# phuang1024/Starst3r

Hardware: AMD Instinct MI355X
Metric: 3DGS train iters/sec @ 1M Gaussians, 8x1080p views (higher is better)
Workload: dtype f32

## Files before the change

### starst3r_amd/csrc/api.hip

```cpp
#include <stdarg.h>

#include "common.h"

static thread_local char g_err[512] = "";

void st3r_set_error(const char* fmt, ...) {
    va_list ap;
    va_start(ap, fmt);
    vsnprintf(g_err, sizeof(g_err), fmt, ap);
    va_end(ap);
}

ST3R_EXPORT int st3r_version(void) { return ST3R_VERSION; }
ST3R_EXPORT const char* st3r_last_error(void) { return g_err; }

ST3R_EXPORT int st3r_ctx_create(int device, st3r_ctx** out) {
    ARG_CHECK(out);
    int ndev = 0;
    HIP_TRY(hipGetDeviceCount(&ndev));
    ARG_CHECK(device >= 0 && device < ndev);
    HIP_TRY(hipSetDevice(device));
    st3r_ctx* c = new (std::nothrow) st3r_ctx();
    if (!c) { st3r_set_error("out of host memory"); return ST3R_ERR_NOMEM; }
    memset(c, 0, sizeof(*c));
// ... 43 lines not shown
    *grown = 0;
    if (bytes == 0) bytes = 16;
    if (ctx->slot_bytes[slot] < bytes) {
        size_t want = bytes + bytes / 4;
        want = (want + 255) & ~(size_t)255;
        if (ctx->slot_ptr[slot]) {
            HIP_TRY(hipDeviceSynchronize());
            HIP_TRY(hipFree(ctx->slot_ptr[slot]));
            ctx->slot_ptr[slot] = nullptr; ctx->slot_bytes[slot] = 0;
        }
        hipError_t e = hipMalloc(&ctx->slot_ptr[slot], want);
        if (e != hipSuccess) {
            st3r_set_error("arena slot %d: hipMalloc(%zu) failed: %s", slot, want, hipGetErrorString(e));
            return ST3R_ERR_NOMEM;
        }
        ctx->slot_bytes[slot] = want;
        *grown = 1;
    }
    *out = ctx->slot_ptr[slot];
    return ST3R_OK;
}

ST3R_EXPORT int st3r_ctx_peek(st3r_ctx* ctx, void* stream, int which, void* dst, int64_t bytes) {
    ARG_CHECK(ctx && dst && bytes >= 0 && which >= 0 && which <= 10);
    static const int slots[11] = {SLOT_VALS_B, SLOT_OFFSETS, SLOT_SPLATS, SLOT_CUM,
                                  SLOT_MCMC_CUM, SLOT_MCMC_DEAD, SLOT_MCMC_SAMPLED, SLOT_MCMC_COUNT,
                                  SLOT_RGB, SLOT_ALPHA, SLOT_COUNTS};
    ARG_CHECK((size_t)bytes <= ctx->slot_bytes[slots[which]]);
    HIP_TRY(hipMemcpyAsync(dst, ctx->slot_ptr[slots[which]], (size_t)bytes, hipMemcpyDeviceToDevice,
                           (hipStream_t)stream));
    return ST3R_OK;
}

static const char* k_stage_names[STG_COUNT] = {"project", "scan", "emit", "sort", "offsets", "blend_fwd", "loss",
                                               "blend_bwd", "project_bwd", "adam", "sort_depth"};

ST3R_EXPORT const char* st3r_stage_name(int stage) {
    return (stage >= 0 && stage < STG_COUNT) ? k_stage_names[stage] : "";
}

static void prof_harvest_slot(st3r_ctx* ctx, int slot) {
    for (int st = 0; st < STG_COUNT; ++st) {
        if (!ctx->prof_used[slot][st]) continue;
        float ms = 0.f;
        if (hipEventSynchronize(ctx->prof_ev[slot][st][1]) == hipSuccess &&
            hipEventElapsedTime(&ms, ctx->prof_ev[slot][st][0], ctx->prof_ev[slot][st][1]) == hipSuccess) {
            ctx->prof_ms[st] += ms; ctx->prof_n[st] += 1;
        }
        ctx->prof_used[slot][st] = 0;
    }
// ... 57 lines not shown
int st3r_project_impl(st3r_ctx* ctx, hipStream_t s, int N, int C, const float* means, const float* quats, const float* scales,
                      const float* opacities, const float* sh, int sh_stride, const float* viewmats, const float* Ks,
                      const float* campos, int width, int height, int tile_size, float eps2d, float near_plane,
                      float far_plane, float radius_clip, float* splats, int32_t* tiles_per_gauss, double* reg_sums,
                      uint64_t* depth_keys, int32_t* depth_vals, int tight, uint32_t key_base, void* rects, int rect32,
                      int reg_overwrite, double* zero_ptr, int zero_n, uint32_t* krange);
int st3r_sort_depth_seg_impl(st3r_ctx* ctx, hipStream_t s, int64_t N, int C, uint32_t* keys_in, int32_t* vals_in,
                             uint32_t* keys_out, int32_t* vals_out, const uint32_t* krange);
int st3r_isect_emit_chain_impl(st3r_ctx* ctx, hipStream_t s, int N, int C, const int32_t* perm, const void* rects,
                               int rect32, int tile_w, int tile_h, uint32_t* tile_keys, int32_t* vals, int64_t cap);
int st3r_records_prepare_impl(hipStream_t s, int N, int C, const float* splats, int tile_size, int tile_w, int tile_h,
                              int tight, int32_t* tiles, uint64_t* depth_keys, int32_t* depth_vals, uint32_t key_base,
                              void* rects, int rect32);
int st3r_isect_offsets32_impl(hipStream_t s, int64_t n_isects, const uint32_t* keys, int C, int tile_w, int tile_h,
                              int32_t* offsets, const int32_t* n_dev);
int st3r_sort_depth_impl(st3r_ctx* ctx, hipStream_t s, int64_t n, int end_bit, uint64_t* keys_in, int32_t* vals_in,
                         uint64_t* keys_out, int32_t* vals_out);
int st3r_sort_depth32_impl(st3r_ctx* ctx, hipStream_t s, int64_t n, int end_bit, uint32_t* keys_in, int32_t* vals_in,
                           uint32_t* keys_out, int32_t* vals_out);
int st3r_sort_tile_impl(st3r_ctx* ctx, hipStream_t s, int64_t n, int end_bit, uint32_t* keys_in, int32_t* vals_in,
                        uint32_t* keys_out, int32_t* vals_out, const int32_t* n_dev);
int st3r_blend_fwd_impl(st3r_ctx* ctx, hipStream_t s, int C, int W, int H, int tile_w, int tile_h,
                        const float* splats, const int32_t* offsets, const int32_t* flat, int64_t n_isects,
                        float* rgb, float* alpha, int32_t* last_ids, bool for_backward, bool end_in_offsets);
int st3r_blend_bwd_impl(st3r_ctx* ctx, hipStream_t s, int C, int W, int H, int tile_w, int tile_h,
                        const float* splats, const int32_t* offsets, const int32_t* flat, int64_t n_isects,
                        const float* alpha, const int32_t* last_ids, const float* v_rgb, const float* v_alpha,
                        const int32_t* cum, const uint64_t* rects, const uint64_t* rectbase, int tight, int64_t n_pairs,
                        float* v_splats,
                        bool end_in_offsets, st3r_vtile_ref* defer);
int st3r_project_sh_bwd_impl(hipStream_t s, int N, int C, const float* means, const float* quats, const float* scales,
                             const float* opacities, const float* sh, int sh_stride, const float* viewmats,
                             const float* Ks, const float* campos, int width, int height, float eps2d,
                             const float* splats, const float* v_splats, float reg_views, float opac_fac,
                             float scale_fac, float* grads, bool accumulate, int g_begin, int g_end, bool range_major,
                             const st3r_vtile_ref* slots);
int st3r_loss_impl(st3r_ctx* ctx, hipStream_t s, int C, int H, int W, const float* render, const float* gt,
                   float w_l1, float w_ssim, double* sums, float* v_render, bool sums_cleared);

static int bit_length_u32(uint32_t v) { int n = 0; while (v) { ++n; v >>= 1; } return n; }

static int settle_pending_count(st3r_ctx* ctx) {
    if (!ctx->count_pending) return ST3R_OK;
    HIP_TRY(hipEventSynchronize(ctx->count_event));
    ctx->count_pending = 0;
    const int64_t n = (int64_t)((int32_t*)(ctx->pinned + 8))[0];
    if (n < 0) {
        ctx->isect_hint = 0;
        ctx->view_chunks = (ctx->view_chunks > 0 ? ctx->view_chunks : 1) * 2;
        st3r_set_error("the previous step produced more than 2^31 tile intersections: its gradients were incomplete -- "
                       "repeat it (st3r_gs_train_fwd_bwd / st3r_gs_train_step now walk the views in %d chunks)",
                       ctx->view_chunks);
        return ST3R_ERR_CAPACITY;
// ... 173 lines not shown
        for (int c = 0; c < C; ++c) loss += w_l1 * sums[2 * c] * inv_px + w_ssim * (1.0 - sums[2 * c + 1] * inv_cnt);
        loss += reg_views * (opac_k * reg_sums[0] + scale_k * reg_sums[1]);
        loss_out[0] = (float)loss;
    }
}

static int train_views(st3r_ctx* ctx, hipStream_t s, int N, int C, const float* means, const float* quats,
                       const float* scales, const float* opacities, const float* sh, int sh_stride,
                       const float* viewmats, const float* Ks, const float* campos, const float* gt_images, int W, int H,
                       float ssim_fac, float opac_fac, float scale_fac, double* sums, double* reg_sums, bool allow_async,
                       bool accumulate, float* grads, RasterOut* ro_out) {
    const int64_t n_pairs = (int64_t)N * C, n_px = (int64_t)C * H * W;
    RasterOut ro;
    int rc = rasterize_front(ctx, s, N, C, means, quats, scales, opacities, sh, sh_stride, viewmats, Ks, campos, W, H,
                             reg_sums, 1, nullptr, allow_async, &ro, sums);
    if (rc) return rc;
    const bool eio = true;
    GET(SLOT_RGB, float, n_px * 3, rgb);
    GET(SLOT_ALPHA, float, n_px, alpha);
    GET(SLOT_LAST, int32_t, n_px, last);
    GET(SLOT_VRENDER, float, n_px * 3, v_rgb);
    float* const v_splats = nullptr;
    st3r_vtile_ref slots_{}; st3r_vtile_ref* const slots = &slots_;
    st3r_prof_begin(ctx, s, STG_BLEND_FWD);
    rc = st3r_blend_fwd_impl(ctx, s, C, W, H, ro.tile_w, ro.tile_h, ro.splats, ro.offsets, ro.flat, ro.n_isects, rgb,
                             alpha, last, true, eio);
    st3r_prof_end(ctx, s, STG_BLEND_FWD);
    if (rc) return rc;
    st3r_prof_begin(ctx, s, STG_LOSS);
    rc = st3r_loss_impl(ctx, s, C, H, W, rgb, gt_images, 1.0f - ssim_fac, ssim_fac, sums, v_rgb, true);
    st3r_prof_end(ctx, s, STG_LOSS);
    if (rc) return rc;
    st3r_prof_begin(ctx, s, STG_BLEND_BWD);
    rc = st3r_blend_bwd_impl(ctx, s, C, W, H, ro.tile_w, ro.tile_h, ro.splats, ro.offsets, ro.flat, ro.n_isects, alpha,
                             last, v_rgb, nullptr, ro.cum, (ctx->debug_flags & 2) ? nullptr : ro.rects,
                             (ctx->debug_flags & 2) ? nullptr : ro.rectbase, 1, n_pairs, v_splats,
                             eio, slots);
    st3r_prof_end(ctx, s, STG_BLEND_BWD);
    if (rc) return rc;
    st3r_prof_begin(ctx, s, STG_PROJECT_BWD);
    ctx->ranges_recorded = 0;
    if (ctx->n_ranges > 1 && ctx->comm_stream) {
        GET(SLOT_GSTAGE, float, (int64_t)23 * N, gstage);
        const int K = ctx->n_ranges;
        for (int j = 0; j < K && !rc; ++j) {
            const int g0 = (int)((int64_t)N * j / K), g1 = (int)((int64_t)N * (j + 1) / K);
            rc = st3r_project_sh_bwd_impl(s, N, C, means, quats, scales, opacities, sh, sh_stride, viewmats, Ks, campos, W,
                                          H, 0.3f, ro.splats, v_splats, (float)C, opac_fac, scale_fac, gstage, accumulate, g0,
                                          g1, true, slots);
            if (!rc) HIP_TRY(hipEventRecord(ctx->ev_range_bwd[j], s));
        }
        if (!rc) ctx->ranges_recorded = K;
    } else {
        rc = st3r_project_sh_bwd_impl(s, N, C, means, quats, scales, opacities, sh, sh_stride, viewmats, Ks, campos, W, H,
                                      0.3f, ro.splats, v_splats, (float)C, opac_fac, scale_fac, grads, accumulate, 0, -1,
                                      false, slots);
    }
    st3r_prof_end(ctx, s, STG_PROJECT_BWD);
    *ro_out = ro;
    return rc;
// ... 65 lines not shown
    ARG_CHECK(ctx && N > 0 && C > 0 && width > 0 && height > 0 && records && gt_images && v_records && loss_out);
    ARG_CHECK(C <= ST3R_MAX_VIEWS && (int64_t)N * C < 2147483647LL);
    hipStream_t s = (hipStream_t)stream;
    const int W = width, H = height;
    const int64_t n_pairs = (int64_t)N * C, n_px = (int64_t)C * H * W;
    GET(SLOT_SMALL, double, 2 * (size_t)C + 8, small);
    double* sums = small;
    double* reg_sums = small + 2 * C;
    HIP_TRY(hipMemsetAsync(reg_sums, 0, sizeof(double) * 4, s));
    st3r_prof_next_step(ctx);
    RasterOut ro;
    int rc = settle_pending_count(ctx);
    if (rc) return rc;
    rc = rasterize_front(ctx, s, N, C, nullptr, nullptr, nullptr, nullptr, nullptr, 0, nullptr, nullptr, nullptr, W, H,
                         nullptr, 1, records, stats_host == nullptr, &ro);
    if (rc == ST3R_SPLIT_VIEWS) rc = ST3R_ERR_INVALID;
    if (rc) return rc;
    GET(SLOT_RGB, float, n_px * 3, rgb);
    GET(SLOT_ALPHA, float, n_px, alpha);
    GET(SLOT_LAST, int32_t, n_px, last);
    GET(SLOT_VRENDER, float, n_px * 3, v_rgb);
    st3r_prof_begin(ctx, s, STG_BLEND_FWD);
    rc = st3r_blend_fwd_impl(ctx, s, C, W, H, ro.tile_w, ro.tile_h, ro.splats, ro.offsets, ro.flat, ro.n_isects, rgb,
                             alpha, last, true, true);
    st3r_prof_end(ctx, s, STG_BLEND_FWD);
    if (rc) return rc;
    st3r_prof_begin(ctx, s, STG_LOSS);
    rc = st3r_loss_impl(ctx, s, C, H, W, rgb, gt_images, 1.0f - ssim_fac, ssim_fac, sums, v_rgb, false);
    st3r_prof_end(ctx, s, STG_LOSS);
    if (rc) return rc;
    st3r_prof_begin(ctx, s, STG_BLEND_BWD);
    rc = st3r_blend_bwd_impl(ctx, s, C, W, H, ro.tile_w, ro.tile_h, ro.splats, ro.offsets, ro.flat, ro.n_isects, alpha,
                             last, v_rgb, nullptr, ro.cum, ro.rects, ro.rectbase, 1, n_pairs, v_records, true, nullptr);
    st3r_prof_end(ctx, s, STG_BLEND_BWD);
    if (rc) return rc;
    const int Hi = H - 10, Wi = W - 10;
    const double cnt = (Hi > 0 && Wi > 0) ? (double)Hi * Wi * 3 : 0.0;
    hipLaunchKernelGGL(k_finalize_loss, dim3(1), dim3(64), 0, s, C, sums, reg_sums, 1.0 / ((double)H * W * 3),
                       cnt > 0 ? 1.0 / cnt : 0.0, (double)(1.0f - ssim_fac), (double)ssim_fac, 0.0, 0.0, 0.0, loss_out);
    LAUNCH_CHECK();
    if (stats_host) {
        stats_host[0] = -1; stats_host[1] = ro.n_records; stats_host[2] = st3r_ctx_arena_bytes(ctx); stats_host[3] = -1;
    }
    return ST3R_OK;
}

ST3R_EXPORT int st3r_gs_render(st3r_ctx* ctx, void* stream, int N, int C, const float* means, const float* quats,
                               const float* scales, const float* opacities, const float* sh, int sh_stride,
                               const float* viewmats, const float* Ks, const float* campos, int width, int height,
                               float* rgb, float* alpha, int64_t* stats_host) {
    ARG_CHECK(ctx && N > 0 && C > 0 && width > 0 && height > 0 && sh_stride >= 12);
    ARG_CHECK(C <= ST3R_MAX_VIEWS && (int64_t)N * C < 2147483647LL);
    ARG_CHECK(means && quats && scales && opacities && sh && viewmats && Ks && campos && rgb && alpha);
    hipStream_t s = (hipStream_t)stream;
    RasterOut ro;
    int rc = settle_pending_count(ctx);
    if (rc) return rc;
    rc = rasterize_front(ctx, s, N, C, means, quats, scales, opacities, sh, sh_stride, viewmats, Ks, campos, width, height,
                         nullptr, 0, nullptr, false, &ro);
    if (rc == ST3R_SPLIT_VIEWS) rc = ST3R_ERR_INVALID;
    if (rc) return rc;
    GET(SLOT_LAST, int32_t, (int64_t)C * height * width, last);
    rc = st3r_blend_fwd_impl(ctx, s, C, width, height, ro.tile_w, ro.tile_h, ro.splats, ro.offsets, ro.flat,
                             ro.n_isects, rgb, alpha, last, false, true);
    if (rc) return rc;
    if (stats_host) {
        stats_host[0] = -1; stats_host[1] = ro.n_records; stats_host[2] = st3r_ctx_arena_bytes(ctx); stats_host[3] = 0;
    }
    return ST3R_OK;
}
```

### starst3r_amd/csrc/common.h

```cpp
#pragma once
#include <hip/hip_runtime.h>
#include <stdint.h>
#include <stdio.h>
#include <string.h>

#include "../../include/st3r.h"

#define ST3R_EXPORT extern "C" __attribute__((visibility("default")))

void st3r_set_error(const char* fmt, ...);

#define HIP_TRY(expr)                                                                              \
    do {                                                                                           \
        hipError_t _e = (expr);                                                                    \
        if (_e != hipSuccess) {                                                                    \
            st3r_set_error("%s:%d: %s -> %s", __FILE__, __LINE__, #expr, hipGetErrorString(_e));   \
            return ST3R_ERR_HIP;                                                                   \
        }                                                                                          \
    } while (0)

#define ARG_CHECK(cond)                                                                    \
    do {                                                                                   \
        if (!(cond)) {                                                                     \
            st3r_set_error("%s:%d: invalid argument: %s", __FILE__, __LINE__, #cond);      \
// ... 28 lines not shown
    SLOT_DKEYS_B,
    SLOT_DVALS_A,
    SLOT_DVALS_B,
    SLOT_CUM_D,
    SLOT_NN_PART,
    SLOT_MCMC_CUM,
    SLOT_MCMC_DEAD,
    SLOT_MCMC_RANK,
    SLOT_MCMC_COUNT,
    SLOT_MCMC_SAMPLED,
    SLOT_MCMC_BINOMS,
    SLOT_REG_PART,
    SLOT_RECTS,
    SLOT_RECTS_D,
    SLOT_RECTBASE,
    SLOT_COUNTS,
    SLOT_PSTAGE,
    SLOT_GSTAGE,
    SLOT_ALIGN_CTL,
    SLOT_PAIR_TOUCH,
    SLOT_KRANGE_PART,
    SLOT_SCAN_CHAIN,
    SLOT_POSE_PART,
    SLOT_COUNT
};

enum Stage {
    STG_PROJECT = 0,
    STG_SCAN,
    STG_EMIT,
    STG_SORT,
    STG_OFFSETS,
    STG_BLEND_FWD,
    STG_LOSS,
    STG_BLEND_BWD,
    STG_PROJECT_BWD,
    STG_ADAM,
    STG_SORT_DEPTH,
    STG_COUNT
};
#define PROF_RING 64
#define ST3R_MAX_RANGES 8

#define ST3R_SPLIT_VIEWS 1000

struct st3r_vtile_ref { const int32_t* cum; const float* vtile; int stamp; unsigned vt_cap; const uint32_t* touch; };
// ... 44 lines not shown
```

### starst3r_amd/csrc/gs_blend.hip

```cpp
#include <type_traits>

#include "common.h"
#include "tile_rect.h"
#include "blend_common.h"



struct TileGeom {
    int lb, cam, i, j, start, end, tx0, ty0;
    bool inside;
    float px, py;
};

__device__ __forceinline__ TileGeom tile_geom(int C, int W, int H, int tile_w, int tile_h,
                                              const int32_t* __restrict__ offsets, int n_isects) {
    TileGeom g;
    const int n_tiles = tile_w * tile_h, total = C * n_tiles;
        g.lb = xcd_remap(blockIdx.x, total, XCD_GROUP(C, n_tiles, tile_w));
    g.cam = g.lb / n_tiles;
    const int tile = g.lb - g.cam * n_tiles;
    const int ty = tile / tile_w, tx = tile - ty * tile_w;
    g.tx0 = tx * 16; g.ty0 = ty * 16;
    const int w = threadIdx.x >> 6, lane = threadIdx.x & 63;
    g.j = g.tx0 + ((w & 1) << 3) + (lane & 7);
// ... 118 lines not shown
        out_rgb[3 * p] = r; out_rgb[3 * p + 1] = gg; out_rgb[3 * p + 2] = b;
        out_alpha[p] = 1.0f - T;
        last_ids[p] = TRAIN ? (cur == 0x7fffffff ? cur : cur - 1) : cur;
    }
    if (tile_nb && threadIdx.x == 0) tile_nb[g.lb] = nb;
}

static int hand_off_buffers(st3r_ctx* ctx, int C, int tile_w, int tile_h, int64_t n_isects, uint64_t** cmask,
                            int64_t* words, int32_t** tile_nb) {
    const int64_t total = (int64_t)C * tile_w * tile_h;
    *words = (n_isects >> 6) + 4 * total + 8;
    void* p;
    int rc = st3r_arena_get(ctx, SLOT_CMASK, sizeof(uint64_t) * 4 * (size_t)*words, &p);
    if (rc) return rc;
    *cmask = (uint64_t*)p;
    rc = st3r_arena_get(ctx, SLOT_TILE_NB, sizeof(int32_t) * (size_t)total, &p);
    if (rc) return rc;
    *tile_nb = (int32_t*)p;
    return ST3R_OK;
}

int st3r_blend_fwd_cells_impl(st3r_ctx* ctx, hipStream_t s, int C, int W, int H, int tile_w, int tile_h,
                              const float* splats, const int32_t* offsets, const int32_t* flat, float* rgb, float* alpha,
                              int32_t* last_ids, uint64_t* cmask, int64_t cmask_words, int32_t* tile_nb);

int st3r_blend_fwd_impl(st3r_ctx* ctx, hipStream_t s, int C, int W, int H, int tile_w, int tile_h,
                        const float* splats, const int32_t* offsets, const int32_t* flat, int64_t n_isects,
                        float* rgb, float* alpha, int32_t* last_ids, bool for_backward, bool end_in_offsets) {
    const int total = C * tile_w * tile_h;
    uint64_t* cmask = nullptr; int64_t words = 0; int32_t* tile_nb = nullptr;
    if (for_backward) {
        int rc = hand_off_buffers(ctx, C, tile_w, tile_h, n_isects, &cmask, &words, &tile_nb);
        if (rc) return rc;
    }
    if ((for_backward && end_in_offsets && !(ctx->debug_flags & 128)) || (end_in_offsets && (ctx->debug_flags & 512)))
        return st3r_blend_fwd_cells_impl(ctx, s, C, W, H, tile_w, tile_h, splats, offsets, flat, rgb, alpha, last_ids, cmask,
                                         words, tile_nb);
    if (for_backward && end_in_offsets)
        hipLaunchKernelGGL(k_blend_fwd<true>, dim3(total), dim3(BLK), 0, s, C, W, H, tile_w, tile_h, (const float4*)splats,
                           offsets, flat, -1, rgb, alpha, last_ids, cmask, words, tile_nb, ctx->debug_flags & 1);
    else
        hipLaunchKernelGGL(k_blend_fwd<false>, dim3(total), dim3(BLK), 0, s, C, W, H, tile_w, tile_h, (const float4*)splats,
                           offsets, flat, end_in_offsets ? -1 : (int)n_isects, rgb, alpha, last_ids, cmask, words, tile_nb,
                           ctx->debug_flags & 1);
    LAUNCH_CHECK();
    return ST3R_OK;
}

ST3R_EXPORT int st3r_gs_blend_fwd(st3r_ctx* ctx, void* stream, int C, int width, int height, int tile_size,
                                  int tile_w, int tile_h, const float* splats, const int32_t* offsets,
                                  const int32_t* flatten_ids, int64_t n_isects, float* rgb, float* alpha,
                                  int32_t* last_ids) {
    ARG_CHECK(ctx && C > 0 && width > 0 && height > 0 && tile_size == 16);
    ARG_CHECK(tile_w == (width + 15) / 16 && tile_h == (height + 15) / 16);
    ARG_CHECK(splats && offsets && rgb && alpha && last_ids && n_isects >= 0 && n_isects < 2147483647LL);
    ARG_CHECK(n_isects == 0 || flatten_ids);
    return st3r_blend_fwd_impl(ctx, (hipStream_t)stream, C, width, height, tile_w, tile_h, splats, offsets,
                               flatten_ids, n_isects, rgb, alpha, last_ids, true, false);
}

__device__ __forceinline__ void bwd_phase2(const float2* __restrict__ pr, unsigned tpack, int cnt, int lane, const float4* sA, float* accw, float qxf_lane, float qyf_lane,
                                           const float (&pvr)[CHUNK], const float (&pvg)[CHUNK],
                                           const float (&pvb)[CHUNK]) {
    static_assert(CHUNK == 4, "one DPP row per record of the chunk");
    const int r = lane >> 4, part = lane & 15;
    wave_lds_sync();
    const int t = (tpack >> (8 * r)) & 0xFF;
    const float2 mean = *reinterpret_cast<const float2*>(&sA[t]);
    const float dy = mean.y - qyf_lane;
    const float2* src = pr + r * PAIR_STRIDE + PAIR_AT(part * CHUNK);
    float W0 = 0.f, W1 = 0.f, W2 = 0.f, Sr = 0.f, Sg = 0.f, Sb = 0.f;
#pragma unroll
    for (int i = 0; i < CHUNK; ++i) {
        const float2 v = src[i];
        W0 += v.x;
        if (i == 1) { W1 = v.x; W2 = v.x; }
        if (i > 1) { W1 = fmaf((float)i, v.x, W1); W2 = fmaf((float)(i * i), v.x, W2); }
        Sr = fmaf(v.y, pvr[i], Sr); Sg = fmaf(v.y, pvg[i], Sg); Sb = fmaf(v.y, pvb[i], Sb);
    }
    const float d0 = mean.x - qxf_lane;
    const float So = W0, Sx = fmaf(d0, W0, -W1), Sxx = fmaf(d0, Sx - W1, W2);
    const float Sy = So * dy, Sxy = Sx * dy, Syy = Sy * dy;
    float k0, k1, k2;
    reduce9_rows(Sx, Sy, So, Sxx, Sxy, Syy, Sr, Sg, Sb, k0, k1, k2);
    if (r < cnt && (lane & 3) == 0) {
        const int b = (lane >> 2) & 3;
        const int slot0 = ((b & 1) << 1) | (b >> 1);
        float* acc = accw + t * ACC_VALS;
        acc[slot0] = k0;
        acc[4 + slot0] = k1;
        if (b == 0) acc[8] = k2;
    }
    wave_lds_sync();
}

template <bool HAS_VA, bool TOUCH = false>
__global__ __launch_bounds__(BLK) __attribute__((amdgpu_waves_per_eu(8))) void k_blend_bwd(int C, int W, int H, int tile_w, int tile_h,
                                                   const float4* __restrict__ splats,
                                                   const int32_t* __restrict__ offsets,
                                                   const int32_t* __restrict__ flat, int n_isects,
                                                   const float* __restrict__ out_alpha,
                                                   const int32_t* __restrict__ last_ids,
                                                   const float* __restrict__ v_rgb,
                                                   const float* __restrict__ v_alpha,
                                                   const uint64_t* __restrict__ cmask, int64_t cmask_words,
                                                   const int32_t* __restrict__ tile_nb,
                                                   const int32_t* __restrict__ cum,
                                                   const uint64_t* __restrict__ rects,
                                                   const uint64_t* __restrict__ rectbase, int tight,
                                                   float* __restrict__ vtile, int stamp, unsigned vt_cap) {

    __shared__ float4 sA[HB];
    __shared__ float4 sB[HB];
    __shared__ float sC[HB];
    __shared__ float sAccW[4][HB * ACC_VALS];
    __shared__ float2 sPair[4][CHUNK * PAIR_STRIDE];
    __shared__ uint64_t sClampW;
    const TileGeom g = tile_geom(C, W, H, tile_w, tile_h, offsets, n_isects);
    const int nb = tile_nb[g.lb];
    if (nb == 0) return;
    const int w = threadIdx.x >> 6, lane = threadIdx.x & 63;
    const int64_t p = ((int64_t)g.cam * H + g.i) * W + g.j;
    float T_final = 1.0f, vr = 0.f, vg = 0.f, vb = 0.f, va = 0.f;
    int bin_final = -1;
    if (g.inside) {
        T_final = 1.0f - out_alpha[p];
        vr = v_rgb[3 * p]; vg = v_rgb[3 * p + 1]; vb = v_rgb[3 * p + 2];
        if (HAS_VA) va = v_alpha[p];
        bin_final = last_ids[p];
    }
    const bool chk_index = __builtin_amdgcn_ballot_w64(bin_final != 0x7fffffff) != 0;
    float2* pr = sPair[w];
    float* accw = sAccW[w];
    float pvr[CHUNK], pvg[CHUNK], pvb[CHUNK];
    const int pbase = (lane & 15) * CHUNK;
    {
        float* px = reinterpret_cast<float*>(pr);
        px[lane] = vr; px[64 + lane] = vg; px[128 + lane] = vb;
        wave_lds_sync();
#pragma unroll
        for (int i = 0; i < CHUNK; ++i) { pvr[i] = px[pbase + i]; pvg[i] = px[64 + pbase + i]; pvb[i] = px[128 + pbase + i]; }
        wave_lds_sync();
    }
    const float qxf = (float)(g.tx0 + ((w & 1) << 3) + (pbase & 7)) + 0.5f;
    const float qyf_part = (float)(g.ty0 + ((w >> 1) << 3) + (pbase >> 3)) + 0.5f;
    float k_big = 0x1p64f, k_neg_thr = -__int_as_float(0x3b808080) * 0x1p64f;
    asm volatile("" : "+v"(k_big), "+v"(k_neg_thr));
    float T = T_final;
    float bv = 0.f;
    const int64_t mbase = mask_base(g.lb, g.start);
    const uint64_t* wmask = cmask + (int64_t)__builtin_amdgcn_readfirstlane(w) * cmask_words + mbase;
    uint64_t m_next = wmask[(BLK / HB) * nb - 1];
    for (int hb = (BLK / HB) * nb - 1; hb >= 0; --hb) {
        const int bs = g.start + hb * HB;
        const int bsz = min(HB, g.end - bs);
        const uint64_t m_cur = m_next;
        if (hb > 0) m_next = wmask[hb - 1];
        if (bsz <= 0) continue;
        int my_u = -1, my_cb = 0;
        float my_op = 0.f, my_ca = 0.f, my_cbb = 0.f, my_cc = 0.f;
        if ((int)threadIdx.x < bsz) {
            const int t = threadIdx.x;
            const int64_t my_id = flat[bs + t];
            const int64_t word = mbase + hb;
#pragma unroll
            for (int ww = 0; ww < 4; ++ww) my_cb |= (int)((cmask[ww * cmask_words + word] >> (t & 63)) & 1ull) << ww;
            float4 a = make_float4(0.f, 0.f, 0.f, 0.f), b = a, c = a;
            if (my_cb)
            {
                a = splats[my_id * 3 + 0];
                b = splats[my_id * 3 + 1];
                c = splats[my_id * 3 + 2];
                sA[t] = make_float4(a.x, a.y, a.z, -0.5f * LOG2E * a.w);
                sB[t] = make_float4(-LOG2E * b.x, -0.5f * LOG2E * b.y, b.z, b.w);
                sC[t] = c.x;
            }
            const float det_ = a.w * b.y - b.x * b.x;
            const bool hard = my_cb && !(a.z <= 0.998f && a.w > 0.f && b.y > 0.f && det_ >= 2e-3f * (a.w * b.y));
            const uint64_t cw = __builtin_amdgcn_ballot_w64(hard);
            if (t == 0) sClampW = cw;
            if (my_cb && rectbase) {
                if (TOUCH) reinterpret_cast<uint32_t*>(const_cast<uint64_t*>(rects))[my_id] = (uint32_t)stamp;
                const uint64_t r = rectbase[my_id];
                const int x0 = (int)(r & 0x3FF), y0 = (int)((r >> 10) & 0x3FF), rw = (int)((r >> 20) & 0x3FF);
                my_u = (int)(r >> 32) + ((g.ty0 >> 4) - y0) * rw + ((g.tx0 >> 4) - x0);
                my_op = a.z; my_ca = a.w; my_cbb = b.x; my_cc = b.y;
            } else if (my_cb) {
                int x0, y0, rw;
                if (rects) {
                    const uint64_t r = rects[my_id];
                    x0 = (int)(r & 0xFFFF); y0 = (int)((r >> 16) & 0xFFFF); rw = (int)((r >> 32) & 0xFFFF);
                } else {
                    TileRect tr = ref_tile_rect(a.x, a.y, (float)__float_as_int(c.z), 16, tile_w, tile_h);
                    if (tight) tr = tight_tile_rect(tr, a.x, a.y, a.z, a.w, b.x, b.y);
                    x0 = tr.x0; y0 = tr.y0; rw = tr.x1 - tr.x0;
                }
                const int cum_excl = my_id == 0 ? 0 : cum[my_id - 1];
                my_u = cum_excl + ((g.ty0 >> 4) - y0) * rw + ((g.tx0 >> 4) - x0);
                my_op = a.z; my_ca = a.w; my_cbb = b.x; my_cc = b.y;
            }
        }
        __syncthreads();
        auto walk = [&](auto chk_tag, auto clamp_tag) {
            constexpr bool CHK = decltype(chk_tag)::value, CLAMP = decltype(clamp_tag)::value;
            uint64_t m = m_cur;
            while (m) {
                unsigned tpack = 0;
                int cnt = 0;
#pragma unroll
                for (int k = 0; k < CHUNK; ++k) {
                    if (m) {
                        const int t = 63 - __builtin_clzll(m);
                        m &= ~(1ull << t);
                        const float4 a = sA[t];
                        const float4 q = sB[t];
                        const float cb_ = sC[t];
                        const float dx = a.x - g.px, dy = a.y - g.py;
                        const float P = blend_power(dx, dy, a.w, q.x, q.y);
                        const float vis0 = __builtin_amdgcn_exp2f(P);
                        const float ov0 = a.z * vis0;
                        float alpha;
                        if (CLAMP) {
                            const float al0 = fminf(0.999f, ov0);
                            uint64_t okm = mask_not_positive(P) & mask_not_less(al0, 1.f / 255.f);
                            if (CHK) okm &= __builtin_amdgcn_ballot_w64(bs + t <= bin_final);
// ... 84 lines not shown
        row[6] = live ? q3.x : 0.f; row[7] = live ? q3.y : 0.f; row[8] = live ? q4.x : 0.f;
        __syncthreads();
        fetch(base + 256 + tid);
        const int lo = max(my_start, base) - base, hi = min(my_end, base + 256) - base;
        for (int r = lo; r < hi; ++r) {
            const float* src = sVal + r * ROW;
#pragma unroll
            for (int k = 0; k < ACC_VALS; ++k) acc[k] += src[k];
        }
        __syncthreads();
    }
    if (tid < np) {
        const int64_t pid = p0 + tid;
        v_splats[pid * 3 + 0] = make_float4(acc[0], acc[1], acc[2], acc[3]);
        v_splats[pid * 3 + 1] = make_float4(acc[4], acc[5], acc[6], acc[7]);
        v_splats[pid * 3 + 2] = make_float4(acc[8], 0.f, 0.f, 0.f);
    }
}

int st3r_blend_bwd_impl(st3r_ctx* ctx, hipStream_t s, int C, int W, int H, int tile_w, int tile_h,
                        const float* splats, const int32_t* offsets, const int32_t* flat, int64_t n_isects,
                        const float* alpha, const int32_t* last_ids, const float* v_rgb, const float* v_alpha,
                        const int32_t* cum, const uint64_t* rects, const uint64_t* rectbase, int tight, int64_t n_pairs,
                        float* v_splats, bool end_in_offsets, st3r_vtile_ref* defer) {
    if (defer) *defer = st3r_vtile_ref{cum, nullptr, 0, 0u, nullptr};
    if (n_isects == 0) {
        if (!defer) HIP_TRY(hipMemsetAsync(v_splats, 0, sizeof(float) * ST3R_SPLAT_STRIDE * (size_t)n_pairs, s));
        return ST3R_OK;
    }
    uint64_t* cmask; int64_t words; int32_t* tile_nb;
    int rc = hand_off_buffers(ctx, C, tile_w, tile_h, n_isects, &cmask, &words, &tile_nb);
    if (rc) return rc;
    void* p; int grown = 0;
    rc = st3r_arena_get2(ctx, SLOT_VTILE, sizeof(float) * VT_STRIDE * (size_t)n_isects, &p, &grown);
    if (rc) return rc;
    float* vtile = (float*)p;
    uint32_t* touch = nullptr;
    int grown_t = 0;
    if (defer && rectbase && !v_alpha && n_isects > 8 * n_pairs) {
        void* pt;
        rc = st3r_arena_get2(ctx, SLOT_PAIR_TOUCH, sizeof(uint32_t) * (size_t)n_pairs, &pt, &grown_t);
        if (rc) return rc;
        touch = (uint32_t*)pt;
    }
    if (grown || ctx->bwd_stamp >= 2147483000) {
        HIP_TRY(hipMemsetAsync(p, 0, ctx->slot_bytes[SLOT_VTILE], s));
        if (ctx->slot_ptr[SLOT_PAIR_TOUCH])
            HIP_TRY(hipMemsetAsync(ctx->slot_ptr[SLOT_PAIR_TOUCH], 0, ctx->slot_bytes[SLOT_PAIR_TOUCH], s));
        ctx->bwd_stamp = 0;
    } else if (grown_t) {
        HIP_TRY(hipMemsetAsync(touch, 0, ctx->slot_bytes[SLOT_PAIR_TOUCH], s));
    }
    const int stamp = ++ctx->bwd_stamp;
    const int total = C * tile_w * tile_h;
    const unsigned vt_cap = (unsigned)(ctx->slot_bytes[SLOT_VTILE] / (sizeof(float) * VT_STRIDE));
    if (v_alpha)
        hipLaunchKernelGGL(k_blend_bwd<true>, dim3(total), dim3(BLK), 0, s, C, W, H, tile_w, tile_h,
                           (const float4*)splats, offsets, flat, end_in_offsets ? -1 : (int)n_isects, alpha, last_ids, v_rgb,
                           v_alpha, cmask, words, tile_nb, cum, rects, rectbase, tight, vtile, stamp, vt_cap);
    else if (touch)
        hipLaunchKernelGGL((k_blend_bwd<false, true>), dim3(total), dim3(BLK), 0, s, C, W, H, tile_w, tile_h,
                           (const float4*)splats, offsets, flat, end_in_offsets ? -1 : (int)n_isects, alpha, last_ids, v_rgb,
                           v_alpha, cmask, words, tile_nb, cum, reinterpret_cast<const uint64_t*>(touch), rectbase, tight, vtile,
                           stamp, vt_cap);
    else
        hipLaunchKernelGGL(k_blend_bwd<false>, dim3(total), dim3(BLK), 0, s, C, W, H, tile_w, tile_h,
                           (const float4*)splats, offsets, flat, end_in_offsets ? -1 : (int)n_isects, alpha, last_ids, v_rgb,
                           v_alpha, cmask, words, tile_nb, cum, rects, rectbase, tight, vtile, stamp, vt_cap);
    LAUNCH_CHECK();
    if (defer) { *defer = st3r_vtile_ref{cum, vtile, stamp, vt_cap, touch}; return ST3R_OK; }
    hipLaunchKernelGGL(k_gather_vtile, dim3(ceil_div(n_pairs, 256)), dim3(256), 0, s, n_pairs, cum, vtile, stamp, vt_cap,
                       (float4*)v_splats);
    LAUNCH_CHECK();
    return ST3R_OK;
}

ST3R_EXPORT int st3r_gs_blend_bwd(st3r_ctx* ctx, void* stream, int C, int width, int height, int tile_size,
                                  int tile_w, int tile_h, const float* splats, const int32_t* offsets,
                                  const int32_t* flatten_ids, int64_t n_isects, const float* alpha,
                                  const int32_t* last_ids, const float* v_rgb, const float* v_alpha,
                                  const int32_t* cum_tiles, int64_t n_pairs, float* v_splats) {
    ARG_CHECK(ctx && C > 0 && width > 0 && height > 0 && tile_size == 16);
    ARG_CHECK(tile_w == (width + 15) / 16 && tile_h == (height + 15) / 16);
    ARG_CHECK(splats && offsets && alpha && last_ids && v_rgb && v_splats && cum_tiles && n_pairs >= 0);
    ARG_CHECK(n_isects >= 0 && n_isects < 2147483647LL && (n_isects == 0 || flatten_ids));
    return st3r_blend_bwd_impl(ctx, (hipStream_t)stream, C, width, height, tile_w, tile_h, splats, offsets,
                               flatten_ids, n_isects, alpha, last_ids, v_rgb, v_alpha, cum_tiles, nullptr, nullptr, 0, n_pairs,
                               v_splats, false, nullptr);
}
```

### starst3r_amd/csrc/gs_blend_cells.hip

```cpp
#include "blend_common.h"
#include <type_traits>

#define CB 256
#define CL_CAP 264
#define SLOT 48
#define SENT_OFF (CB * SLOT)

__device__ __forceinline__ uint2 build_wave_lists(const uint16_t* sCm, uint16_t* myList, int cell, int lane) {
    const int idx = lane & 15;
    const uint4 d0 = *reinterpret_cast<const uint4*>(sCm + 16 * idx);
    const uint4 d1 = *reinterpret_cast<const uint4*>(sCm + 16 * idx + 8);
    const unsigned sent2 = (unsigned)SENT_OFF | ((unsigned)SENT_OFF << 16);
    const uint4 sv = make_uint4(sent2, sent2, sent2, sent2);
    *reinterpret_cast<uint4*>(myList + 16 * idx) = sv;
    *reinterpret_cast<uint4*>(myList + 16 * idx + 8) = sv;
    const unsigned dw[8] = {d0.x, d0.y, d0.z, d0.w, d1.x, d1.y, d1.z, d1.w};
    unsigned piece = 0;
#pragma unroll
    for (int j = 0; j < 8; ++j) {
        piece |= ((dw[j] >> cell) & 1u) << (2 * j);
        piece |= ((dw[j] >> (cell + 16)) & 1u) << (2 * j + 1);
    }
    const unsigned cnt = __builtin_popcount(piece);
    unsigned inc = cnt;
// ... 48 lines not shown
    int lb, cam, tx0, ty0, start, end, i, j, cell;
    bool inside;
};

__device__ __forceinline__ CellTile cell_tile(int C, int W, int H, int tile_w, int tile_h, const int32_t* __restrict__ offsets) {
    CellTile g;
    const int n_tiles = tile_w * tile_h, total = C * n_tiles;
    g.lb = xcd_remap(blockIdx.x, total, XCD_GROUP(C, n_tiles, tile_w));
    g.cam = g.lb / n_tiles;
    const int tile = g.lb - g.cam * n_tiles;
    const int ty = tile / tile_w, tx = tile - ty * tile_w;
    g.tx0 = tx * 16; g.ty0 = ty * 16;
    const int w = threadIdx.x >> 6, lane = threadIdx.x & 63, rho = lane >> 4, idx = lane & 15;
    const int cx = ((w & 1) << 1) | (rho & 1), cy = ((w >> 1) << 1) | (rho >> 1);
    g.cell = cy * 4 + cx;
    g.j = g.tx0 + 4 * cx + (idx & 3);
    g.i = g.ty0 + 4 * cy + (idx >> 2);
    g.inside = (g.i < H) && (g.j < W);
    g.start = offsets[g.lb];
    g.end = offsets[g.lb + 1];
    return g;
}

__global__ __launch_bounds__(BLK) __attribute__((amdgpu_waves_per_eu(7))) void k_blend_fwd_cells(int C, int W, int H, int tile_w, int tile_h,
                                                         const float4* __restrict__ splats,
                                                         const int32_t* __restrict__ offsets,
                                                         const int32_t* __restrict__ flat,
                                                         float* __restrict__ out_rgb, float* __restrict__ out_alpha,
                                                         int32_t* __restrict__ last_ids,
                                                         uint64_t* __restrict__ cmask, int64_t cmask_words,
                                                         int32_t* __restrict__ tile_nb, int no_cull) {
    __shared__ float4 sR[(CB + 1) * (SLOT / 16)];
    __shared__ uint16_t sList[16][CL_CAP];
    __shared__ uint16_t sCm[BLK];
    __shared__ unsigned sFlag[CB];
    __shared__ int sHard[2];
    const CellTile g = cell_tile(C, W, H, tile_w, tile_h, offsets);
    const int w = threadIdx.x >> 6, lane = threadIdx.x & 63;
    CellPx s;
    s.px = (float)g.j + 0.5f; s.py = (float)g.i + 0.5f;
    s.thr = g.inside ? 1.f / 255.f : __builtin_inff();
    s.T = 1.0f; s.r = s.g = s.b = 0.f; s.cur = 0x7fffffff;
    if (threadIdx.x < SLOT / 16) sR[CB * (SLOT / 16) + threadIdx.x] = make_float4(0.f, 0.f, 0.f, 0.f);
    if (threadIdx.x < 2) sHard[threadIdx.x] = 0;
    char* sRb = reinterpret_cast<char*>(sR);
    uint16_t* lp = sList[g.cell];
    unsigned char* my_flags = reinterpret_cast<unsigned char*>(sFlag) + w;
    const int64_t mbase = mask_base(g.lb, g.start);
    auto flags_out = [&](int nbp) {
        const unsigned f = sFlag[threadIdx.x];
        const uint64_t c0 = __builtin_amdgcn_ballot_w64((f & 0x000000FFu) != 0), c1 = __builtin_amdgcn_ballot_w64((f & 0x0000FF00u) != 0);
        const uint64_t c2 = __builtin_amdgcn_ballot_w64((f & 0x00FF0000u) != 0), c3 = __builtin_amdgcn_ballot_w64((f & 0xFF000000u) != 0);
        if (cmask && lane == 0) {
            uint64_t* dst = cmask + mbase + nbp * 4 + w;
            dst[0] = c0; dst[cmask_words] = c1; dst[2 * cmask_words] = c2; dst[3 * cmask_words] = c3;
        }
    };
    int nb = 0;
    int id_next = g.start + (int)threadIdx.x < g.end ? flat[g.start + threadIdx.x] : 0;
    for (int bs = g.start; bs < g.end; bs += CB, ++nb) {
        const int idx = bs + threadIdx.x;
        const bool have = idx < g.end;
        float4 ra = make_float4(0.f, 0.f, 0.f, 0.f), rb = ra, rc = ra;
        unsigned cm = 0;
        const int64_t id = id_next;
        if (idx + CB < g.end) id_next = flat[idx + CB];
        bool hard = false;
        if (have) {
            ra = splats[id * 3 + 0]; rb = splats[id * 3 + 1]; rc = splats[id * 3 + 2];
            hard = !(ra.z <= 0.998f && ra.w > 0.f && rb.y > 0.f && (ra.w * rb.y - rb.x * rb.x) >= 2e-3f * (ra.w * rb.y));
            cm = no_cull ? 0xFFFFu : cell_mask16(ra.x, ra.y, ra.z, ra.w, rb.x, rb.y, g.tx0, g.ty0);
        }
        if (__syncthreads_and(s.thr > 1.0f)) break;
        if (nb > 0) flags_out(nb - 1);
        {
            float4* slot = sR + threadIdx.x * (SLOT / 16);
            slot[0] = make_float4(ra.x, ra.y, ra.z, -0.5f * LOG2E * ra.w);
            slot[1] = make_float4(-LOG2E * rb.x, -0.5f * LOG2E * rb.y, rb.z, rb.w);
            slot[2] = make_float4(rc.x, 0.f, 0.f, 0.f);
        }
        sCm[threadIdx.x] = (uint16_t)cm;
        sFlag[threadIdx.x] = 0u;
        if (__builtin_amdgcn_ballot_w64(hard) != 0 && lane == 0) sHard[nb & 1] = 1;
        if (threadIdx.x == 0) sHard[(nb + 1) & 1] = 0;
        __syncthreads();
        if (__builtin_amdgcn_ballot_w64(s.thr < 1.0f) != 0) {
            const uint2 lens = build_wave_lists(sCm, lp, g.cell, lane);
            const int l0 = lens.x & 0xFFFF, l1 = lens.x >> 16, l2 = lens.y & 0xFFFF, l3 = lens.y >> 16;
            auto windows = [&](auto lean_tag) {
            constexpr bool LEAN = decltype(lean_tag)::value;
            uint2 e = *reinterpret_cast<const uint2*>(lp);
            for (int k0 = 0;; k0 += 32) {
                const uint64_t live = __builtin_amdgcn_ballot_w64(s.thr < 1.0f);
// ... 35 lines not shown
                        const unsigned ee = *reinterpret_cast<const unsigned*>(lp + k0 + p2);
                        if (two & 1u) my_flags[4 * (((ee & 0xFFFFu) >> 4) * 43691u >> 17)] = 1;
                        if (two & 2u) my_flags[4 * (((ee >> 16) >> 4) * 43691u >> 17)] = 1;
                    }
                }
            }
            };
            if (__builtin_amdgcn_readfirstlane(sHard[nb & 1]) == 0) windows(std::true_type{}); else windows(std::false_type{});
        }
    }
    __syncthreads();
    if (nb > 0) flags_out(nb - 1);
    if (g.inside) {
        const int64_t p = ((int64_t)g.cam * H + g.i) * W + g.j;
        out_rgb[3 * p] = s.r; out_rgb[3 * p + 1] = s.g; out_rgb[3 * p + 2] = s.b;
        out_alpha[p] = 1.0f - s.T;
        last_ids[p] = s.cur == 0x7fffffff ? s.cur : s.cur - 1;
    }
    if (tile_nb && threadIdx.x == 0) tile_nb[g.lb] = nb;
}

int st3r_blend_fwd_cells_impl(st3r_ctx* ctx, hipStream_t s, int C, int W, int H, int tile_w, int tile_h,
                              const float* splats, const int32_t* offsets, const int32_t* flat, float* rgb, float* alpha,
                              int32_t* last_ids, uint64_t* cmask, int64_t cmask_words, int32_t* tile_nb) {
    const int total = C * tile_w * tile_h;
    hipLaunchKernelGGL(k_blend_fwd_cells, dim3(total), dim3(BLK), 0, s, C, W, H, tile_w, tile_h, (const float4*)splats,
                       offsets, flat, rgb, alpha, last_ids, cmask, cmask_words, tile_nb, ctx->debug_flags & 1);
    LAUNCH_CHECK();
    return ST3R_OK;
}
```

Baseline: 188.7.

## Stage per-intersection splat records in forward blend for sequential backward reads

The forward cell-blend kernel now writes a contiguous 48-byte record per intersection to a new arena slot. Each record holds the splat conic/color data, the precomputed vtile index, the hard flag and the id. The backward blend kernel reads this stream sequentially instead of gathering through flat ids and splats, and it no longer recomputes the rect-derived index. This trades extra forward writes and 12 floats per intersection of memory for coalesced backward loads. An optional LDS prefetch path sits behind a compile-time macro.

```diff
diff --git a/starst3r_amd/csrc/api.hip b/starst3r_amd/csrc/api.hip
--- a/starst3r_amd/csrc/api.hip
+++ b/starst3r_amd/csrc/api.hip
@@ -89,10 +89,10 @@
 }
 
 ST3R_EXPORT int st3r_ctx_peek(st3r_ctx* ctx, void* stream, int which, void* dst, int64_t bytes) {
-    ARG_CHECK(ctx && dst && bytes >= 0 && which >= 0 && which <= 10);
-    static const int slots[11] = {SLOT_VALS_B, SLOT_OFFSETS, SLOT_SPLATS, SLOT_CUM,
+    ARG_CHECK(ctx && dst && bytes >= 0 && which >= 0 && which <= 11);
+    static const int slots[12] = {SLOT_VALS_B, SLOT_OFFSETS, SLOT_SPLATS, SLOT_CUM,
                                   SLOT_MCMC_CUM, SLOT_MCMC_DEAD, SLOT_MCMC_SAMPLED, SLOT_MCMC_COUNT,
-                                  SLOT_RGB, SLOT_ALPHA, SLOT_COUNTS};
+                                  SLOT_RGB, SLOT_ALPHA, SLOT_COUNTS, SLOT_VTILE};
     ARG_CHECK((size_t)bytes <= ctx->slot_bytes[slots[which]]);
     HIP_TRY(hipMemcpyAsync(dst, ctx->slot_ptr[slots[which]], (size_t)bytes, hipMemcpyDeviceToDevice,
                            (hipStream_t)stream));
@@ -196,13 +196,14 @@
                         uint32_t* keys_out, int32_t* vals_out, const int32_t* n_dev);
 int st3r_blend_fwd_impl(st3r_ctx* ctx, hipStream_t s, int C, int W, int H, int tile_w, int tile_h,
                         const float* splats, const int32_t* offsets, const int32_t* flat, int64_t n_isects,
-                        float* rgb, float* alpha, int32_t* last_ids, bool for_backward, bool end_in_offsets);
+                        float* rgb, float* alpha, int32_t* last_ids, bool for_backward, bool end_in_offsets,
+                        const uint64_t* rectbase, float* stream);
 int st3r_blend_bwd_impl(st3r_ctx* ctx, hipStream_t s, int C, int W, int H, int tile_w, int tile_h,
                         const float* splats, const int32_t* offsets, const int32_t* flat, int64_t n_isects,
                         const float* alpha, const int32_t* last_ids, const float* v_rgb, const float* v_alpha,
                         const int32_t* cum, const uint64_t* rects, const uint64_t* rectbase, int tight, int64_t n_pairs,
                         float* v_splats,
-                        bool end_in_offsets, st3r_vtile_ref* defer);
+                        bool end_in_offsets, st3r_vtile_ref* defer, const float* stream);
 int st3r_project_sh_bwd_impl(hipStream_t s, int N, int C, const float* means, const float* quats, const float* scales,
                              const float* opacities, const float* sh, int sh_stride, const float* viewmats,
                              const float* Ks, const float* campos, int width, int height, float eps2d,
@@ -422,9 +423,14 @@
     GET(SLOT_VRENDER, float, n_px * 3, v_rgb);
     float* const v_splats = nullptr;
     st3r_vtile_ref slots_{}; st3r_vtile_ref* const slots = &slots_;
+    float* stream = nullptr;
+    if (ro.rectbase && ro.n_isects > 0 && !(ctx->debug_flags & (4096 | 128 | 2))) {
+        GET(SLOT_BLEND_STREAM, float, 12 * ro.n_isects, st);
+        stream = st;
+    }
     st3r_prof_begin(ctx, s, STG_BLEND_FWD);
     rc = st3r_blend_fwd_impl(ctx, s, C, W, H, ro.tile_w, ro.tile_h, ro.splats, ro.offsets, ro.flat, ro.n_isects, rgb,
-                             alpha, last, true, eio);
+                             alpha, last, true, eio, ro.rectbase, stream);
     st3r_prof_end(ctx, s, STG_BLEND_FWD);
     if (rc) return rc;
     st3r_prof_begin(ctx, s, STG_LOSS);
@@ -435,7 +441,7 @@
     rc = st3r_blend_bwd_impl(ctx, s, C, W, H, ro.tile_w, ro.tile_h, ro.splats, ro.offsets, ro.flat, ro.n_isects, alpha,
                              last, v_rgb, nullptr, ro.cum, (ctx->debug_flags & 2) ? nullptr : ro.rects,
                              (ctx->debug_flags & 2) ? nullptr : ro.rectbase, 1, n_pairs, v_splats,
-                             eio, slots);
+                             eio, slots, stream);
     st3r_prof_end(ctx, s, STG_BLEND_BWD);
     if (rc) return rc;
     st3r_prof_begin(ctx, s, STG_PROJECT_BWD);
@@ -547,7 +553,7 @@
     GET(SLOT_VRENDER, float, n_px * 3, v_rgb);
     st3r_prof_begin(ctx, s, STG_BLEND_FWD);
     rc = st3r_blend_fwd_impl(ctx, s, C, W, H, ro.tile_w, ro.tile_h, ro.splats, ro.offsets, ro.flat, ro.n_isects, rgb,
-                             alpha, last, true, true);
+                             alpha, last, true, true, nullptr, nullptr);
     st3r_prof_end(ctx, s, STG_BLEND_FWD);
     if (rc) return rc;
     st3r_prof_begin(ctx, s, STG_LOSS);
@@ -556,7 +562,7 @@
     if (rc) return rc;
     st3r_prof_begin(ctx, s, STG_BLEND_BWD);
     rc = st3r_blend_bwd_impl(ctx, s, C, W, H, ro.tile_w, ro.tile_h, ro.splats, ro.offsets, ro.flat, ro.n_isects, alpha,
-                             last, v_rgb, nullptr, ro.cum, ro.rects, ro.rectbase, 1, n_pairs, v_records, true, nullptr);
+                             last, v_rgb, nullptr, ro.cum, ro.rects, ro.rectbase, 1, n_pairs, v_records, true, nullptr, nullptr);
     st3r_prof_end(ctx, s, STG_BLEND_BWD);
     if (rc) return rc;
     const int Hi = H - 10, Wi = W - 10;
@@ -587,7 +593,7 @@
     if (rc) return rc;
     GET(SLOT_LAST, int32_t, (int64_t)C * height * width, last);
     rc = st3r_blend_fwd_impl(ctx, s, C, width, height, ro.tile_w, ro.tile_h, ro.splats, ro.offsets, ro.flat,
-                             ro.n_isects, rgb, alpha, last, false, true);
+                             ro.n_isects, rgb, alpha, last, false, true, nullptr, nullptr);
     if (rc) return rc;
     if (stats_host) {
         stats_host[0] = -1; stats_host[1] = ro.n_records; stats_host[2] = st3r_ctx_arena_bytes(ctx); stats_host[3] = 0;
diff --git a/starst3r_amd/csrc/common.h b/starst3r_amd/csrc/common.h
--- a/starst3r_amd/csrc/common.h
+++ b/starst3r_amd/csrc/common.h
@@ -74,6 +74,7 @@
     SLOT_KRANGE_PART,
     SLOT_SCAN_CHAIN,
     SLOT_POSE_PART,
+    SLOT_BLEND_STREAM,
     SLOT_COUNT
 };
 
diff --git a/starst3r_amd/csrc/gs_blend.hip b/starst3r_amd/csrc/gs_blend.hip
--- a/starst3r_amd/csrc/gs_blend.hip
+++ b/starst3r_amd/csrc/gs_blend.hip
@@ -164,11 +164,13 @@
 
 int st3r_blend_fwd_cells_impl(st3r_ctx* ctx, hipStream_t s, int C, int W, int H, int tile_w, int tile_h,
                               const float* splats, const int32_t* offsets, const int32_t* flat, float* rgb, float* alpha,
-                              int32_t* last_ids, uint64_t* cmask, int64_t cmask_words, int32_t* tile_nb);
+                              int32_t* last_ids, uint64_t* cmask, int64_t cmask_words, int32_t* tile_nb,
+                              const uint64_t* rectbase, float* stream);
 
 int st3r_blend_fwd_impl(st3r_ctx* ctx, hipStream_t s, int C, int W, int H, int tile_w, int tile_h,
                         const float* splats, const int32_t* offsets, const int32_t* flat, int64_t n_isects,
-                        float* rgb, float* alpha, int32_t* last_ids, bool for_backward, bool end_in_offsets) {
+                        float* rgb, float* alpha, int32_t* last_ids, bool for_backward, bool end_in_offsets,
+                        const uint64_t* rectbase, float* stream) {
     const int total = C * tile_w * tile_h;
     uint64_t* cmask = nullptr; int64_t words = 0; int32_t* tile_nb = nullptr;
     if (for_backward) {
@@ -177,7 +179,11 @@
     }
     if ((for_backward && end_in_offsets && !(ctx->debug_flags & 128)) || (end_in_offsets && (ctx->debug_flags & 512)))
         return st3r_blend_fwd_cells_impl(ctx, s, C, W, H, tile_w, tile_h, splats, offsets, flat, rgb, alpha, last_ids, cmask,
-                                         words, tile_nb);
+                                         words, tile_nb, rectbase, for_backward ? stream : nullptr);
+    if (stream) {
+        st3r_set_error("blend forward: a staging stream needs the cell-list kernel");
+        return ST3R_ERR_INVALID;
+    }
     if (for_backward && end_in_offsets)
         hipLaunchKernelGGL(k_blend_fwd<true>, dim3(total), dim3(BLK), 0, s, C, W, H, tile_w, tile_h, (const float4*)splats,
                            offsets, flat, -1, rgb, alpha, last_ids, cmask, words, tile_nb, ctx->debug_flags & 1);
@@ -198,7 +204,7 @@
     ARG_CHECK(splats && offsets && rgb && alpha && last_ids && n_isects >= 0 && n_isects < 2147483647LL);
     ARG_CHECK(n_isects == 0 || flatten_ids);
     return st3r_blend_fwd_impl(ctx, (hipStream_t)stream, C, width, height, tile_w, tile_h, splats, offsets,
-                               flatten_ids, n_isects, rgb, alpha, last_ids, true, false);
+                               flatten_ids, n_isects, rgb, alpha, last_ids, true, false, nullptr, nullptr);
 }
 
 __device__ __forceinline__ void bwd_phase2(const float2* __restrict__ pr, unsigned tpack, int cnt, int lane, const float4* sA, float* accw, float qxf_lane, float qyf_lane,
@@ -236,7 +242,7 @@
     wave_lds_sync();
 }
 
-template <bool HAS_VA, bool TOUCH = false>
+template <bool HAS_VA, bool TOUCH = false, bool STREAM = false>
 __global__ __launch_bounds__(BLK) __attribute__((amdgpu_waves_per_eu(8))) void k_blend_bwd(int C, int W, int H, int tile_w, int tile_h,
                                                    const float4* __restrict__ splats,
                                                    const int32_t* __restrict__ offsets,
@@ -250,7 +256,8 @@
                                                    const int32_t* __restrict__ cum,
                                                    const uint64_t* __restrict__ rects,
                                                    const uint64_t* __restrict__ rectbase, int tight,
-                                                   float* __restrict__ vtile, int stamp, unsigned vt_cap) {
+                                                   float* __restrict__ vtile, int stamp, unsigned vt_cap,
+                                                   const float4* __restrict__ stream) {
 
     __shared__ float4 sA[HB];
     __shared__ float4 sB[HB];
@@ -258,6 +265,9 @@
     __shared__ float sAccW[4][HB * ACC_VALS];
     __shared__ float2 sPair[4][CHUNK * PAIR_STRIDE];
     __shared__ uint64_t sClampW;
+#if BLEND_BWD_PREFETCH
+    __shared__ float sTouch[64];
+#endif
     const TileGeom g = tile_geom(C, W, H, tile_w, tile_h, offsets, n_isects);
     const int nb = tile_nb[g.lb];
     if (nb == 0) return;
@@ -301,7 +311,25 @@
         if (bsz <= 0) continue;
         int my_u = -1, my_cb = 0;
         float my_op = 0.f, my_ca = 0.f, my_cbb = 0.f, my_cc = 0.f;
-        if ((int)threadIdx.x < bsz) {
+        if (STREAM && (int)threadIdx.x < bsz) {
+            const int t = threadIdx.x;
+            const float4* e = stream + (int64_t)(bs + t) * 3;
+            const int64_t word = mbase + hb;
+#pragma unroll
+            for (int ww = 0; ww < 4; ++ww) my_cb |= (int)((cmask[ww * cmask_words + word] >> (t & 63)) & 1ull) << ww;
+            float4 a = make_float4(0.f, 0.f, 0.f, 0.f), b = a, c = a;
+            if (!TOUCH || my_cb) { a = e[0]; b = e[1]; c = e[2]; }
+            if (my_cb) {
+                sA[t] = make_float4(a.x, a.y, a.z, -0.5f * LOG2E * a.w);
+                sB[t] = make_float4(-LOG2E * b.x, -0.5f * LOG2E * b.y, b.z, b.w);
+                sC[t] = c.x;
+                if (TOUCH) reinterpret_cast<uint32_t*>(const_cast<uint64_t*>(rects))[__float_as_int(c.w)] = (uint32_t)stamp;
+                my_u = __float_as_int(c.y);
+                my_op = a.z; my_ca = a.w; my_cbb = b.x; my_cc = b.y;
+            }
+            const uint64_t cw = __builtin_amdgcn_ballot_w64(my_cb && __float_as_int(c.z) != 0);
+            if (t == 0) sClampW = cw;
+        } else if (!STREAM && (int)threadIdx.x < bsz) {
             const int t = threadIdx.x;
             const int64_t my_id = flat[bs + t];
             const int64_t word = mbase + hb;
@@ -343,6 +371,13 @@
             }
         }
         __syncthreads();
+#if BLEND_BWD_PREFETCH
+        if (STREAM && hb > 0 && threadIdx.x < 64) {
+            const char* src = reinterpret_cast<const char*>(stream + (int64_t)(bs - HB) * 3) + 48 * threadIdx.x;
+            __builtin_amdgcn_global_load_lds((__attribute__((address_space(1))) void*)src,
+                                             (__attribute__((address_space(3))) void*)sTouch, 4, 0, 0);
+        }
+#endif
         auto walk = [&](auto chk_tag, auto clamp_tag) {
             constexpr bool CHK = decltype(chk_tag)::value, CLAMP = decltype(clamp_tag)::value;
             uint64_t m = m_cur;
@@ -473,7 +508,7 @@
                         const float* splats, const int32_t* offsets, const int32_t* flat, int64_t n_isects,
                         const float* alpha, const int32_t* last_ids, const float* v_rgb, const float* v_alpha,
                         const int32_t* cum, const uint64_t* rects, const uint64_t* rectbase, int tight, int64_t n_pairs,
-                        float* v_splats, bool end_in_offsets, st3r_vtile_ref* defer) {
+                        float* v_splats, bool end_in_offsets, st3r_vtile_ref* defer, const float* stream) {
     if (defer) *defer = st3r_vtile_ref{cum, nullptr, 0, 0u, nullptr};
     if (n_isects == 0) {
         if (!defer) HIP_TRY(hipMemsetAsync(v_splats, 0, sizeof(float) * ST3R_SPLAT_STRIDE * (size_t)n_pairs, s));
@@ -505,19 +540,29 @@
     const int stamp = ++ctx->bwd_stamp;
     const int total = C * tile_w * tile_h;
     const unsigned vt_cap = (unsigned)(ctx->slot_bytes[SLOT_VTILE] / (sizeof(float) * VT_STRIDE));
+    const float4* const st = (const float4*)stream;
     if (v_alpha)
         hipLaunchKernelGGL(k_blend_bwd<true>, dim3(total), dim3(BLK), 0, s, C, W, H, tile_w, tile_h,
                            (const float4*)splats, offsets, flat, end_in_offsets ? -1 : (int)n_isects, alpha, last_ids, v_rgb,
-                           v_alpha, cmask, words, tile_nb, cum, rects, rectbase, tight, vtile, stamp, vt_cap);
+                           v_alpha, cmask, words, tile_nb, cum, rects, rectbase, tight, vtile, stamp, vt_cap, nullptr);
+    else if (touch && st)
+        hipLaunchKernelGGL((k_blend_bwd<false, true, true>), dim3(total), dim3(BLK), 0, s, C, W, H, tile_w, tile_h,
+                           (const float4*)splats, offsets, flat, end_in_offsets ? -1 : (int)n_isects, alpha, last_ids, v_rgb,
+                           v_alpha, cmask, words, tile_nb, cum, reinterpret_cast<const uint64_t*>(touch), rectbase, tight, vtile,
+                           stamp, vt_cap, st);
     else if (touch)
         hipLaunchKernelGGL((k_blend_bwd<false, true>), dim3(total), dim3(BLK), 0, s, C, W, H, tile_w, tile_h,
                            (const float4*)splats, offsets, flat, end_in_offsets ? -1 : (int)n_isects, alpha, last_ids, v_rgb,
                            v_alpha, cmask, words, tile_nb, cum, reinterpret_cast<const uint64_t*>(touch), rectbase, tight, vtile,
-                           stamp, vt_cap);
+                           stamp, vt_cap, nullptr);
+    else if (st)
+        hipLaunchKernelGGL((k_blend_bwd<false, false, true>), dim3(total), dim3(BLK), 0, s, C, W, H, tile_w, tile_h,
+                           (const float4*)splats, offsets, flat, end_in_offsets ? -1 : (int)n_isects, alpha, last_ids, v_rgb,
+                           v_alpha, cmask, words, tile_nb, cum, rects, rectbase, tight, vtile, stamp, vt_cap, st);
     else
         hipLaunchKernelGGL(k_blend_bwd<false>, dim3(total), dim3(BLK), 0, s, C, W, H, tile_w, tile_h,
                            (const float4*)splats, offsets, flat, end_in_offsets ? -1 : (int)n_isects, alpha, last_ids, v_rgb,
-                           v_alpha, cmask, words, tile_nb, cum, rects, rectbase, tight, vtile, stamp, vt_cap);
+                           v_alpha, cmask, words, tile_nb, cum, rects, rectbase, tight, vtile, stamp, vt_cap, nullptr);
     LAUNCH_CHECK();
     if (defer) { *defer = st3r_vtile_ref{cum, vtile, stamp, vt_cap, touch}; return ST3R_OK; }
     hipLaunchKernelGGL(k_gather_vtile, dim3(ceil_div(n_pairs, 256)), dim3(256), 0, s, n_pairs, cum, vtile, stamp, vt_cap,
@@ -537,5 +582,5 @@
     ARG_CHECK(n_isects >= 0 && n_isects < 2147483647LL && (n_isects == 0 || flatten_ids));
     return st3r_blend_bwd_impl(ctx, (hipStream_t)stream, C, width, height, tile_w, tile_h, splats, offsets,
                                flatten_ids, n_isects, alpha, last_ids, v_rgb, v_alpha, cum_tiles, nullptr, nullptr, 0, n_pairs,
-                               v_splats, false, nullptr);
-}
+                               v_splats, false, nullptr, nullptr);
+}
diff --git a/starst3r_amd/csrc/gs_blend_cells.hip b/starst3r_amd/csrc/gs_blend_cells.hip
--- a/starst3r_amd/csrc/gs_blend_cells.hip
+++ b/starst3r_amd/csrc/gs_blend_cells.hip
@@ -94,6 +94,7 @@
     return g;
 }
 
+template <bool STREAM>
 __global__ __launch_bounds__(BLK) __attribute__((amdgpu_waves_per_eu(7))) void k_blend_fwd_cells(int C, int W, int H, int tile_w, int tile_h,
                                                          const float4* __restrict__ splats,
                                                          const int32_t* __restrict__ offsets,
@@ -101,7 +102,9 @@
                                                          float* __restrict__ out_rgb, float* __restrict__ out_alpha,
                                                          int32_t* __restrict__ last_ids,
                                                          uint64_t* __restrict__ cmask, int64_t cmask_words,
-                                                         int32_t* __restrict__ tile_nb, int no_cull) {
+                                                         int32_t* __restrict__ tile_nb, int no_cull,
+                                                         const uint64_t* __restrict__ rectbase,
+                                                         float4* __restrict__ stream) {
     __shared__ float4 sR[(CB + 1) * (SLOT / 16)];
     __shared__ uint16_t sList[16][CL_CAP];
     __shared__ uint16_t sCm[BLK];
@@ -140,7 +143,17 @@
         bool hard = false;
         if (have) {
             ra = splats[id * 3 + 0]; rb = splats[id * 3 + 1]; rc = splats[id * 3 + 2];
+            uint64_t rr = 0;
+            if (STREAM) rr = rectbase[id];
             hard = !(ra.z <= 0.998f && ra.w > 0.f && rb.y > 0.f && (ra.w * rb.y - rb.x * rb.x) >= 2e-3f * (ra.w * rb.y));
+            if (STREAM) {
+                const int x0 = (int)(rr & 0x3FF), y0 = (int)((rr >> 10) & 0x3FF), rw = (int)((rr >> 20) & 0x3FF);
+                const int u = (int)(rr >> 32) + ((g.ty0 >> 4) - y0) * rw + ((g.tx0 >> 4) - x0);
+                float4* e = stream + (int64_t)idx * 3;
+                e[0] = ra;
+                e[1] = rb;
+                e[2] = make_float4(rc.x, __int_as_float(u), __int_as_float(hard ? 1 : 0), __int_as_float((int)id));
+            }
             cm = no_cull ? 0xFFFFu : cell_mask16(ra.x, ra.y, ra.z, ra.w, rb.x, rb.y, g.tx0, g.ty0);
         }
         if (__syncthreads_and(s.thr > 1.0f)) break;
@@ -222,10 +235,17 @@
 
 int st3r_blend_fwd_cells_impl(st3r_ctx* ctx, hipStream_t s, int C, int W, int H, int tile_w, int tile_h,
                               const float* splats, const int32_t* offsets, const int32_t* flat, float* rgb, float* alpha,
-                              int32_t* last_ids, uint64_t* cmask, int64_t cmask_words, int32_t* tile_nb) {
+                              int32_t* last_ids, uint64_t* cmask, int64_t cmask_words, int32_t* tile_nb,
+                              const uint64_t* rectbase, float* stream) {
     const int total = C * tile_w * tile_h;
-    hipLaunchKernelGGL(k_blend_fwd_cells, dim3(total), dim3(BLK), 0, s, C, W, H, tile_w, tile_h, (const float4*)splats,
-                       offsets, flat, rgb, alpha, last_ids, cmask, cmask_words, tile_nb, ctx->debug_flags & 1);
+    if (stream)
+        hipLaunchKernelGGL(k_blend_fwd_cells<true>, dim3(total), dim3(BLK), 0, s, C, W, H, tile_w, tile_h,
+                           (const float4*)splats, offsets, flat, rgb, alpha, last_ids, cmask, cmask_words, tile_nb,
+                           ctx->debug_flags & 1, rectbase, (float4*)stream);
+    else
+        hipLaunchKernelGGL(k_blend_fwd_cells<false>, dim3(total), dim3(BLK), 0, s, C, W, H, tile_w, tile_h,
+                           (const float4*)splats, offsets, flat, rgb, alpha, last_ids, cmask, cmask_words, tile_nb,
+                           ctx->debug_flags & 1, nullptr, nullptr);
     LAUNCH_CHECK();
     return ST3R_OK;
 }
```

Measured after the change: 180.5, median of 2. 4.3% lower.
